# SimonMacLean/NeRF-or-nothing

Hardware: AMD Instinct MI355X
Metric: train rays/sec (128 samples/ray, 8×256 MLP) at 1/2/4/8 MI355X; PSNR vs ref (higher is better)
Workload: dtype f32; 1 GPU; BASELINE configs[1]: 1024-ray global batch x 128+128 samples, 8x256 MLP fwd/bwd + Adam; global_batch=1024, rays_per_gpu=1024, micro_batch=1024, parallelism=dp1, precision=f32

## Files before the change

nerf-or-nothing_amd/csrc/kernels/mlp16.h:

```cpp
#pragma once
#include "mlp_common.h"

namespace nof {

constexpr int kMlp16Threads = 512;
constexpr int kIpe16Floats = 6 * 64 * 4;

__device__ __forceinline__ f32x4 mfma16(float a, float b, f32x4 c) {
  return __builtin_amdgcn_mfma_f32_16x16x4f32(a, b, c, 0, 0, 0);
}

__device__ __forceinline__ void slice16_dma_step(const float* __restrict__ src, float* dst, int tid, int i) {
  const int wave = tid >> 6;
  const __amdgpu_buffer_rsrc_t rsrc =
      __builtin_amdgcn_make_buffer_rsrc(const_cast<float*>(src), (short)0, 0x7fffffff, 0x00020000);
  __builtin_amdgcn_raw_ptr_buffer_load_lds(rsrc, (lptr_t)(dst + (kMlp16Threads * i + 64 * wave) * 4), 16, tid * 16,
                                           i * kMlp16Threads * 16, 0, 0);
}
__device__ __forceinline__ void slice16_dma(const float* __restrict__ src, float* dst, int tid) {
#pragma unroll
  for (int i = 0; i < 4; ++i) slice16_dma_step(src, dst, tid, i);
}

template <int P> constexpr int ring16_slots() { return P == 0 ? 4 : 3; }
template <int P> constexpr int ring16_floats() { return ring16_slots<P>() * kSliceFloats; }
__device__ __forceinline__ void ring16_prologue(const float* __restrict__ img, float* lds, int tid) {
  slice16_dma(img, lds, tid);
  slice16_dma(img + kSliceFloats, lds + kSliceFloats, tid);
}

__device__ __forceinline__ constexpr int feat16(int t, int g, int r) { return 16 * t + 4 * g + r; }

constexpr int kStoreNT = 2;
struct BlkStore16 {
  static constexpr bool kHalf = false;
  uint32_t voff[4];
  __device__ __forceinline__ BlkStore16(int lane, int half) {
    const int g = lane >> 4, s = 16 * half + (lane & 15);
#pragma unroll
    for (int r = 0; r < 4; ++r)
      voff[r] = 512u * g + ((((s >> 2) ^ (4 * (g & 1) + r)) << 4) | ((s & 3) << 2));
  }
  __device__ __forceinline__ void store(__amdgpu_buffer_rsrc_t blk, int t, int r, float v) const {
    __builtin_amdgcn_raw_buffer_store_b32(__float_as_uint(v), blk, (int)voff[r], 2048 * t + 128 * r, kStoreNT);
  }
};
__device__ __forceinline__ __amdgpu_buffer_rsrc_t blk_rsrc(float* blk) {
  return __builtin_amdgcn_make_buffer_rsrc(blk, (short)0, 0x7fffffff, 0x00020000);
}

template <bool kNT>
struct BlkStore16H {
  static constexpr bool kHalf = true;
  uint32_t voff;
  uint32_t voff2;
  uint32_t sel;
  __device__ __forceinline__ BlkStore16H(int lane, int half) {
    const int g = lane >> 4, j = lane & 15;
    voff = 256u * g + ((((2 * half + (j >> 3)) ^ g) << 4) | ((j & 7) << 1));
    voff2 = 256u * g + 64u * (j & 1) + ((((2 * half + (j >> 3)) ^ g) << 4) | ((j & 6) << 1));
    sel = (j & 1) ? 0x03020706u : 0x05040100u;
  }
  __device__ __forceinline__ void store_pairs(__amdgpu_buffer_rsrc_t blk, int t, uint32_t p01, uint32_t p23) const {
    const uint32_t q01 = (uint32_t)__builtin_amdgcn_mov_dpp((int)p01, 0xB1, 0xF, 0xF, false);
    const uint32_t q23 = (uint32_t)__builtin_amdgcn_mov_dpp((int)p23, 0xB1, 0xF, 0xF, false);
    __builtin_amdgcn_raw_buffer_store_b32(__builtin_amdgcn_perm(q01, p01, sel), blk, (int)voff2, 1024 * t,
                                          kNT ? kStoreNT : 0);
    __builtin_amdgcn_raw_buffer_store_b32(__builtin_amdgcn_perm(q23, p23, sel), blk, (int)voff2 + 128, 1024 * t,
                                          kNT ? kStoreNT : 0);
  }
  __device__ __forceinline__ void store(__amdgpu_buffer_rsrc_t blk, int t, int r, float v) const {
    store_h(blk, t, r, (_Float16)v);
  }
  __device__ __forceinline__ void store_h(__amdgpu_buffer_rsrc_t blk, int t, int r, _Float16 h) const {
    __builtin_amdgcn_raw_buffer_store_b16(__builtin_bit_cast(unsigned short, h), blk, (int)voff + 64 * r, 1024 * t,
                                          kNT ? kStoreNT : 0);
  }
};
template <int P, bool kBwd> struct Store16 { typedef BlkStore16 T; typedef float E; };
template <bool kBwd> struct Store16<2, kBwd> { typedef BlkStore16H<true> T; typedef _Float16 E; };
template <class E>
__device__ __forceinline__ __amdgpu_buffer_rsrc_t blk_rsrc_t(E* blk) {
  return __builtin_amdgcn_make_buffer_rsrc(blk, (short)0, 0x7fffffff, 0x00020000);
}

__device__ __forceinline__ uint2* mask16_ptr(uint32_t* masks, int blk, int slot, int half, int lane) {
  return reinterpret_cast<uint2*>(mask_ptr(masks, blk, slot) + half * 128) + lane;
}
__device__ __forceinline__ bool mask16_bit(const uint2& m, int t, int r) {
  return ((t >> 3 ? m.y : m.x) >> (31 - ((t & 7) * 4 + r))) & 1u;
}
__device__ __forceinline__ float mask16_apply(const uint2& m, int t, int r, float v) {
  const uint32_t w = t >> 3 ? m.y : m.x;
  uint32_t all;
  asm("v_bfe_i32 %0, %1, %2, 1" : "=v"(all) : "v"(w), "n"(31 - ((t & 7) * 4 + r)));
  return __uint_as_float(__float_as_uint(v) & all);
}

__device__ __forceinline__ float relu_bit(float z, uint32_t& mw) {
  const int h = max(__float_as_int(z), 0);
  asm volatile("v_cmp_lt_i32 vcc, 0, %1\n\tv_addc_co_u32 %0, vcc, %0, %0, vcc" : "+v"(mw) : "v"(h) : "vcc");
  return __int_as_float(h);
}

__device__ __forceinline__ void split4h(const float (&x)[4], uint32_t& hi01, uint32_t& hi23, uint32_t& lo01,
                                        uint32_t& lo23) {
  typedef _Float16 h2 __attribute__((ext_vector_type(2)));
  typedef float f2 __attribute__((ext_vector_type(2)));
  hi01 = __builtin_bit_cast(uint32_t, __builtin_convertvector((f2{x[0], x[1]}), h2));
  hi23 = __builtin_bit_cast(uint32_t, __builtin_convertvector((f2{x[2], x[3]}), h2));
  float r[4];
  asm("v_fma_mix_f32 %0, %1, 1.0, -%2 op_sel_hi:[0,0,1]" : "=v"(r[0]) : "v"(x[0]), "v"(hi01));
  asm("v_fma_mix_f32 %0, %1, 1.0, -%2 op_sel:[0,0,1] op_sel_hi:[0,0,1]" : "=v"(r[1]) : "v"(x[1]), "v"(hi01));
  asm("v_fma_mix_f32 %0, %1, 1.0, -%2 op_sel_hi:[0,0,1]" : "=v"(r[2]) : "v"(x[2]), "v"(hi23));
  asm("v_fma_mix_f32 %0, %1, 1.0, -%2 op_sel:[0,0,1] op_sel_hi:[0,0,1]" : "=v"(r[3]) : "v"(x[3]), "v"(hi23));
  lo01 = __builtin_bit_cast(uint32_t, __builtin_convertvector((f2{r[0], r[1]}), h2));
  lo23 = __builtin_bit_cast(uint32_t, __builtin_convertvector((f2{r[2], r[3]}), h2));
}

template <bool kSplit, bool kStore, class ST>
__device__ __forceinline__ void put_tile(float (&bin)[16][4], int t, const float (&v)[4], const ST& bst,
                                         __amdgpu_buffer_rsrc_t blk) {
  if constexpr (kSplit) {
    uint32_t hi01, hi23, lo01, lo23;
    split4h(v, hi01, hi23, lo01, lo23);
    const int row = t & ~1, c = 2 * (t & 1);
    bin[row][c] = __uint_as_float(hi01);
    bin[row][c + 1] = __uint_as_float(hi23);
    bin[row + 1][c] = __uint_as_float(lo01);
    bin[row + 1][c + 1] = __uint_as_float(lo23);
    if constexpr (kStore) {
      if constexpr (ST::kHalf) {
        bst.store_pairs(blk, t, hi01, hi23);
      } else {
#pragma unroll
        for (int r = 0; r < 4; ++r) bst.store(blk, t, r, v[r]);
      }
    }
  } else {
#pragma unroll
    for (int r = 0; r < 4; ++r) {
      bin[t][r] = v[r];
      if constexpr (kStore) bst.store(blk, t, r, v[r]);
    }
  }
}

struct NoEpi16 {
  static constexpr int kVmPerPart = 0;
  __device__ __forceinline__ void operator()(int) {}
};

template <int NT_B, int NT_I, int OT, int kSlots, class Epi>
__device__ __forceinline__ void mlp_layer16(const float (&bin)[16][4], const float* ipe, f32x4 (&acc)[16],
                                            float* lds, int& cur, const float*& wsrc, bool last_in_schedule, int tid,
                                            int lane, Epi& epi, const float* cinit) {
  static_assert(OT % 2 == 0 && OT <= 16, "row tiles come in pairs");
  constexpr int NG = OT;
  constexpr int kEpiGroup1 = 4;
  constexpr int kEpiGroup2 = (NG / 2 + 4 < NG) ? NG / 2 + 4 : NG - 1;
  const int g = lane >> 4;
  const int row = lane & 15;
  const int swz = (row >> 1) & 7;
#pragma unroll
  for (int t = 0; t < NT_B + NT_I; ++t) {
    const bool dma = !(last_in_schedule && t + 2 >= NT_B + NT_I);
    const int nxt2 = kSlots == 4 ? ((cur + 2) & 3) : (cur == 0 ? 2 : cur - 1);
    const float* W = lds + cur * kSliceFloats + row * 32;
    auto aread = [&](int q, int which) {
      const int tt = q / (OT / 2), p = q % (OT / 2);
      return *reinterpret_cast<const f32x4*>(W + (2 * p + which) * 16 * 32 + (((4 * tt + g) ^ swz) << 2));
    };
    f32x4 a0 = aread(0, 0), a1 = aread(0, 1);
    auto cread = [&](int p, int which) { return *reinterpret_cast<const f32x4*>(cinit + 16 * (2 * p + which)); };
    f32x4 c0 = {}, c1 = {};
    if (t == 0 && cinit) { c0 = cread(0, 0); c1 = cread(0, 1); }
#pragma unroll
    for (int q = 0; q < NG; ++q) {
      const int tt = q / (OT / 2), p = q % (OT / 2);
      f32x4 b4;
      if (t < NT_B) {
        const int tb = (t < NT_B) ? 2 * t + tt : 0;
        b4[0] = bin[tb][0]; b4[1] = bin[tb][1]; b4[2] = bin[tb][2]; b4[3] = bin[tb][3];
      } else {
        const int ti = (t >= NT_B) ? 2 * (t - NT_B) + tt : 0;
        if constexpr (kSlots == 4) {
          b4[0] = ipe[4 * ti]; b4[1] = ipe[4 * ti + 1]; b4[2] = ipe[4 * ti + 2]; b4[3] = ipe[4 * ti + 3];
        } else b4 = *reinterpret_cast<const f32x4*>(ipe + (ti * 64 + lane) * 4);
      }
      asm volatile("" ::"v"(a0), "v"(a1), "v"(c0), "v"(c1));
      f32x4 n0 = a0, n1 = a1, m0 = c0, m1 = c1;
      if (q + 1 < NG) {
        n0 = aread(q + 1, 0);
        n1 = aread(q + 1, 1);
      }
      if (t == 0 && cinit && q + 1 < OT / 2) { m0 = cread(q + 1, 0); m1 = cread(q + 1, 1); }
      if (dma && q < 4) slice16_dma_step(wsrc + 2 * kSliceFloats, lds + nxt2 * kSliceFloats, tid, q);
      __builtin_amdgcn_sched_barrier(0);
      const bool first = t == 0 && tt == 0;
#pragma unroll
      for (int r = 0; r < 4; ++r) {
        acc[2 * p] = mfma16(a0[r], b4[r], (first && r == 0) ? c0 : acc[2 * p]);
        acc[2 * p + 1] = mfma16(a1[r], b4[r], (first && r == 0) ? c1 : acc[2 * p + 1]);
      }
      if (t + 1 < NT_B && q == kEpiGroup1) epi(2 * t + 2);
      if (t + 1 < NT_B && q == kEpiGroup2) epi(2 * t + 3);
      __builtin_amdgcn_sched_barrier(0);
      a0 = n0;
      a1 = n1;
      c0 = m0;
      c1 = m1;
    }
    if constexpr (kSlots == 4) {
      if (cur & 1) slice_barrier(t + 1 < NT_B ? 2 * Epi::kVmPerPart : 0);
      cur = (cur + 1) & 3;
    } else {
      slice_barrier((dma ? 4 : 0) + (t + 1 < NT_B ? 2 * Epi::kVmPerPart : 0));
      cur = cur == 2 ? 0 : cur + 1;
    }
    wsrc += kSliceFloats;
  }
}
template <int NT_B, int NT_I, int OT, class Epi>
__device__ __forceinline__ void mlp_layer16h(const float (&bin)[16][4], const float* ipe_lds, f32x4 (&acc)[16],
                                             float* lds, int& cur, const float*& wsrc, bool last_in_schedule, int tid,
                                             int lane, Epi& epi, const float* cinit) {
  typedef SplitMode<2> SM;
  static_assert(OT % 2 == 0 && OT <= 16, "row tiles come in pairs");
  constexpr int kPieces = 2;
  constexpr int kPP0 = 0;
  constexpr int kDmaSteps = 4;
  constexpr int kSlots = ring16_slots<2>();
  constexpr int NG = OT / 2;
  constexpr int kE1 = NG > 4 ? 4 : NG - 1;
  constexpr int kE2 = NG > 6 ? 6 : NG - 1;
#pragma unroll
  for (int t = 0; t < NT_B + NT_I; ++t) {
    const bool dma = !(last_in_schedule && t + 2 >= NT_B + NT_I);
    const int nxt2 = kSlots == 4 ? ((cur + 2) & 3) : (cur == 0 ? 2 : cur - 1);
    const f16x8* W = reinterpret_cast<const f16x8*>(lds + cur * kSliceFloats) + lane;
    Frag<2> b;
    float v[8];
    if (t < NT_B) {
      const int tb = t < NT_B ? 2 * t : 0;
      const f32x4 hi = {bin[tb][0], bin[tb][1], bin[tb][2], bin[tb][3]};
      const f32x4 lo = {bin[tb + 1][0], bin[tb + 1][1], bin[tb + 1][2], bin[tb + 1][3]};
      b.p[0] = __builtin_bit_cast(f16x8, hi);
      b.p[1] = __builtin_bit_cast(f16x8, lo);
    } else {
      const int ti = t >= NT_B ? 2 * (t - NT_B) : 0;
      if constexpr (kSlots == 4) {
#pragma unroll
        for (int i = 0; i < 8; ++i) v[i] = ipe_lds[4 * ti + i];
      } else {
        const f32x4 u0 = *reinterpret_cast<const f32x4*>(ipe_lds + (ti * 64 + lane) * 4);
        const f32x4 u1 = *reinterpret_cast<const f32x4*>(ipe_lds + ((ti + 1) * 64 + lane) * 4);
#pragma unroll
        for (int i = 0; i < 4; ++i) { v[i] = u0[i]; v[4 + i] = u1[i]; }
      }
      split8<2>(v, b);
    }
    Frag<2> a0, a1;
#pragma unroll
    for (int p = 0; p < kPieces; ++p) { a0.p[p] = W[(16 * p) * 64]; a1.p[p] = W[(16 * p + 1) * 64]; }
    auto cread = [&](int rt) { return *reinterpret_cast<const f32x4*>(cinit + 16 * rt); };
    f32x4 c0 = {}, c1 = {};
    if (t == 0 && cinit) { c0 = cread(0); c1 = cread(1); }
#pragma unroll
    for (int q = 0; q < NG; ++q) {
      if constexpr (kPieces == 2) asm volatile("" ::"v"(a0.p[0]), "v"(a0.p[1]), "v"(a1.p[0]), "v"(a1.p[1]), "v"(c0), "v"(c1));
      else asm volatile("" ::"v"(a0.p[0]), "v"(a1.p[0]), "v"(c0), "v"(c1));
      Frag<2> n0 = a0, n1 = a1;
      f32x4 m0 = c0, m1 = c1;
      if (t == 0 && cinit && q + 1 < NG) { m0 = cread(2 * q + 2); m1 = cread(2 * q + 3); }
      if (q + 1 < NG) {
#pragma unroll
        for (int p = 0; p < kPieces; ++p) {
          n0.p[p] = W[(16 * p + 2 * q + 2) * 64];
          n1.p[p] = W[(16 * p + 2 * q + 3) * 64];
        }
      }
      if (dma && q < kDmaSteps) slice16_dma_step(wsrc + 2 * kSliceFloats, lds + nxt2 * kSliceFloats, tid, q);
      __builtin_amdgcn_sched_barrier(0);
      const bool first = t == 0;
#pragma unroll
      for (int pp = kPP0; pp < SM::NPROD; ++pp) {
        acc[2 * q] = SM::mfma16(a0.p[SM::pa(pp)], b.p[SM::pb(pp)], (first && pp == kPP0) ? c0 : acc[2 * q]);
        acc[2 * q + 1] = SM::mfma16(a1.p[SM::pa(pp)], b.p[SM::pb(pp)], (first && pp == kPP0) ? c1 : acc[2 * q + 1]);
      }
      if (t + 1 < NT_B && q == kE1) epi(2 * t + 2);
      if (t + 1 < NT_B && q == kE2) epi(2 * t + 3);
      __builtin_amdgcn_sched_barrier(0);
      a0 = n0;
      a1 = n1;
      c0 = m0;
      c1 = m1;
    }
    if constexpr (kSlots == 4) {
      if (cur & 1) slice_barrier(t + 1 < NT_B ? 2 * Epi::kVmPerPart : 0);
      cur = (cur + 1) & 3;
    } else {
      slice_barrier((dma ? kDmaSteps : 0) + (t + 1 < NT_B ? 2 * Epi::kVmPerPart : 0));
      cur = cur == 2 ? 0 : cur + 1;
    }
    wsrc += kSliceFloats;
  }
}

template <int P, int NT_B, int NT_I, int OT, class Epi>
__device__ __forceinline__ void layer16(const float (&bin)[16][4], const float* ipe_lds, f32x4 (&acc)[16], float* lds,
                                        int& cur, const float*& wsrc, bool last_in_schedule, int tid, int lane,
                                        Epi& epi, const float* cinit = nullptr) {
  if constexpr (P == 2 || P == 3)
    mlp_layer16h<NT_B, NT_I, OT>(bin, ipe_lds, acc, lds, cur, wsrc, last_in_schedule, tid, lane, epi, cinit);
  else
    mlp_layer16<NT_B, NT_I, OT, ring16_slots<P>()>(bin, ipe_lds, acc, lds, cur, wsrc, last_in_schedule, tid, lane,
                                                   epi, cinit);
}
template <int P, int NT_B, int NT_I, int OT>
__device__ __forceinline__ void layer16(const float (&bin)[16][4], const float* ipe_lds, f32x4 (&acc)[16], float* lds,
                                        int& cur, const float*& wsrc, bool last_in_schedule, int tid, int lane,
                                        const float* cinit = nullptr) {
  NoEpi16 none;
  layer16<P, NT_B, NT_I, OT>(bin, ipe_lds, acc, lds, cur, wsrc, last_in_schedule, tid, lane, none, cinit);
}

}
```

nerf-or-nothing_amd/csrc/kernels/mlp_bwd16.hip:

```cpp
#include "common.h"
#include "launch.h"
#include "mlp16.h"

namespace nof {


template <bool kDensity, class ST, bool kSplit = false>
struct BwdEpi16 {
  static constexpr int kVmPerPart = 4;
  const f32x4 (&acc)[16];
  float (&bin)[16][4];
  const ST& bst;
  const int g;
  const float* w8;
  float dzs;
  __amdgpu_buffer_rsrc_t dst_blk;
  uint2 mk;
  f32x4 wnext;

  __device__ __forceinline__ BwdEpi16(const f32x4 (&acc_)[16], float (&bin_)[16][4], const ST& bst_, int lane)
      : acc(acc_), bin(bin_), bst(bst_), g(lane >> 4) {}
  template <class E>
  __device__ __forceinline__ void begin(const uint2* mask, E* dst_blk_, const float* w8_ = nullptr, float dzs_ = 0.0f) {
    mk = *mask;
    dst_blk = blk_rsrc_t(dst_blk_);
    if constexpr (kDensity) {
      w8 = w8_ + 4 * g;
      dzs = dzs_;
      wnext = *reinterpret_cast<const f32x4*>(w8);
    }
  }
  __device__ __forceinline__ void operator()(int t) {
    f32x4 w4;
    if constexpr (kDensity) {
      w4 = wnext;
      if (t + 1 < 16) wnext = *reinterpret_cast<const f32x4*>(w8 + 16 * (t + 1));
    }
    float v[4];
#pragma unroll
    for (int r = 0; r < 4; ++r) {
      v[r] = acc[t][r];
      if constexpr (kDensity) v[r] = __builtin_fmaf(w4[r], dzs, v[r]);
      v[r] = mask16_apply(mk, t, r, v[r]);
    }
    put_tile<kSplit, true>(bin, t, v, bst, dst_blk);
  }
  __device__ __forceinline__ void tile01() {
    (*this)(0);
    (*this)(1);
  }
};

template <int P>
__global__ __launch_bounds__(kMlp16Threads, 1) void k_mlp_bwd16(BwdArgs a0) {
  typedef typename Store16<P, true>::T ST;
  typedef typename Store16<P, true>::E AE;
  __shared__ __attribute__((aligned(16))) float lds[ring16_floats<P>() + 256];
  float* w8_lds = lds + ring16_floats<P>();
  const int tid = threadIdx.x, lane = tid & 63, g = lane >> 4, j = lane & 15;
  const int wave = __builtin_amdgcn_readfirstlane(tid >> 6);
  const int half = wave & 1;
  const ST bst(lane, half);
  const int wg0 = (a0.M / kBlk + 3) / 4;
  const bool second = a0.M1 > 0 && (int)blockIdx.x >= wg0;
  struct {
    int M;
    const float *dsigma, *drgb, *zhead;
    const uint32_t *amax, *masks;
    const float* wimg_b;
    float dbias, rgb_scale;
    float *delta, *delta9x;
  } a;
  a.M = second ? a0.M1 : a0.M;
  a.dsigma = second ? a0.dsigma1 : a0.dsigma;
  a.drgb = second ? a0.drgb1 : a0.drgb;
  a.zhead = second ? a0.zhead1 : a0.zhead;
  a.amax = second ? a0.amax1 : a0.amax;
  a.masks = second ? a0.masks1 : a0.masks;
  a.delta = second ? a0.delta1 : a0.delta;
  a.delta9x = second ? a0.delta9x1 : a0.delta9x;
  a.wimg_b = a0.wimg_b; a.dbias = a0.dbias; a.rgb_scale = a0.rgb_scale;
  const int wg = second ? (int)blockIdx.x - wg0 : (int)blockIdx.x;
  const int nblk = a.M / kBlk;
  const int blk_raw = wg * 4 + (wave >> 1);
  const int blk = blk_raw < nblk ? blk_raw : nblk - 1;
  const int m = blk * kBlk + 16 * half + j;
  NOF_DCHECK(a.M % kBlk == 0 && blk >= 0 && blk < nblk, kChkMlpBlock);
  const float* tail = a.wimg_b + (size_t)kBwdSlices * kSliceFloats;
  const size_t layer_stride = (size_t)nblk * kWidth * kBlk;
  uint32_t* masks = const_cast<uint32_t*>(a.masks);

  const f32x4 zh = reinterpret_cast<const f32x4*>(a.zhead)[m];
  const float dsig = a.dsigma[m];
  const float drgb3[3] = {a.drgb[(size_t)m * 3], a.drgb[(size_t)m * 3 + 1], a.drgb[(size_t)m * 3 + 2]};
  float sc = 1.0f;
  if constexpr (P >= 2) sc = delta_scale(a.amax, false);
  const uint2 mk9 = *mask16_ptr(masks, blk, 8, half, lane);
  f32x4 w10r[8][3];
#pragma unroll
  for (int t = 0; t < 8; ++t)
#pragma unroll
    for (int c = 0; c < 3; ++c)
      w10r[t][c] = *reinterpret_cast<const f32x4*>(tail + kBwdTailW10 + 128 * c + 16 * t + 4 * g);
  const f32x4 w8r = reinterpret_cast<const f32x4*>(tail + kBwdTailW8)[lane];
  __builtin_amdgcn_sched_barrier(0);
  ring16_prologue(a.wimg_b, lds, tid);
  __builtin_amdgcn_sched_barrier(0);

  float dzs = dsig * sigmoid_f(zh[0] + a.dbias);
  float dzc[3];
#pragma unroll
  for (int c = 0; c < 3; ++c) {
    const float s = sigmoid_f(zh[1 + c]);
    dzc[c] = drgb3[c] * (s * (1.0f - s)) * a.rgb_scale;
  }
  if constexpr (P >= 2) {
    dzs *= sc;
#pragma unroll
    for (int c = 0; c < 3; ++c) dzc[c] *= sc;
  }
  if (wave == 0) reinterpret_cast<f32x4*>(w8_lds)[lane] = w8r;
  const __amdgpu_buffer_rsrc_t d9 = blk_rsrc_t(reinterpret_cast<AE*>(a.delta9x) + (size_t)blk * kD9F * kBlk);
#pragma unroll
  for (int r = 0; r < 4; ++r) bst.store(d9, 8, r, g == 0 ? (r == 0 ? dzs : dzc[r - 1]) : 0.0f);
  float bin[16][4];
#pragma unroll
  for (int t = 0; t < 8; ++t) {
    float v[4];
#pragma unroll
    for (int r = 0; r < 4; ++r)
      v[r] = mask16_apply(mk9, t, r, __builtin_fmaf(w10r[t][2][r], dzc[2],
                                                   __builtin_fmaf(w10r[t][1][r], dzc[1], w10r[t][0][r] * dzc[0])));
    put_tile<P >= 2, true>(bin, t, v, bst, d9);
  }
  constexpr int kD9Stores = 4 + 8 * (P == 2 ? 2 : 4);
  static_assert(kD9Stores == (P == 2 ? 20 : 36), "the literals in the waits below");
  if constexpr (P == 2) asm volatile("s_waitcnt vmcnt(20)\n\ts_waitcnt lgkmcnt(0)\n\ts_barrier" ::: "memory");
  else asm volatile("s_waitcnt vmcnt(36)\n\ts_waitcnt lgkmcnt(0)\n\ts_barrier" ::: "memory");

  int cur = 0;
  const float* wsrc = a.wimg_b;
  f32x4 accA[16], accB[16];
  AE* delta_blk = reinterpret_cast<AE*>(a.delta) + (size_t)blk * kWidth * kBlk;
  BwdEpi16<true, ST, P >= 2> e7(accA, bin, bst, lane);
  e7.begin(mask16_ptr(masks, blk, 7, half, lane), delta_blk + 7 * layer_stride, w8_lds, dzs);
  layer16<P, 4, 0, 16>(bin, nullptr, accA, lds, cur, wsrc, false, tid, lane);
  e7.tile01();
  BwdEpi16<false, ST, P >= 2> ea(accA, bin, bst, lane), eb(accB, bin, bst, lane);
  eb.begin(mask16_ptr(masks, blk, 6, half, lane), delta_blk + 6 * layer_stride);
  layer16<P, 8, 0, 16>(bin, nullptr, accB, lds, cur, wsrc, false, tid, lane, e7);
  eb.tile01();
  static_assert(kDepth == 8, "bwd pairing assumes 8 trunk layers");
  for (int l = kDepth - 2; l >= 2; l -= 2) {
    ea.begin(mask16_ptr(masks, blk, l - 1, half, lane), delta_blk + (l - 1) * layer_stride);
    layer16<P, 8, 0, 16>(bin, nullptr, accA, lds, cur, wsrc, false, tid, lane, eb);
    ea.tile01();
    eb.begin(mask16_ptr(masks, blk, l - 2, half, lane), delta_blk + (l - 2) * layer_stride);
    layer16<P, 8, 0, 16>(bin, nullptr, accB, lds, cur, wsrc, l == 2, tid, lane, ea);
    eb.tile01();
  }
#pragma unroll
  for (int t = 2; t < 16; ++t) eb(t);
}

hipError_t launch_mlp_bwd16(const BwdArgs& a, hipStream_t st) {
  const dim3 grid((a.M / kBlk + 3) / 4 + (a.M1 > 0 ? (a.M1 / kBlk + 3) / 4 : 0));
  if (a.split == 2) hipLaunchKernelGGL(k_mlp_bwd16<2>, grid, dim3(kMlp16Threads), 0, st, a);
  else if (a.split == 3) hipLaunchKernelGGL(k_mlp_bwd16<3>, grid, dim3(kMlp16Threads), 0, st, a);
  else hipLaunchKernelGGL(k_mlp_bwd16<0>, grid, dim3(kMlp16Threads), 0, st, a);
  return hipGetLastError();
}

NOF_CHECK_UNIT(check_unit_mlp_bwd16)

}
```

nerf-or-nothing_amd/csrc/kernels/mlp_fwd16.hip:

```cpp
#include "common.h"
#include "geometry.h"
#include "launch.h"
#include "mlp16.h"

namespace nof {


template <bool store, bool kDensity, int NT, class ST, bool kSplit = false>
struct FwdEpi16 {
  static constexpr int kVmPerPart = store ? 4 : 0;
  const f32x4 (&acc)[16];
  float (&bin)[16][4];
  const ST& bst;
  const int g;
  const float* w8;
  __amdgpu_buffer_rsrc_t act_blk;
  uint2* mask_dst;
  uint32_t mw[2];
  f32x4 wnext;
  float zs;

  __device__ __forceinline__ FwdEpi16(const f32x4 (&acc_)[16], float (&bin_)[16][4], const ST& bst_, int lane)
      : acc(acc_), bin(bin_), bst(bst_), g(lane >> 4) {}
  template <class E>
  __device__ __forceinline__ void begin(E* act_blk_, uint2* mask_dst_, const float* w8_ = nullptr) {
    act_blk = blk_rsrc_t(act_blk_);
    mask_dst = mask_dst_;
    mw[0] = mw[1] = 0u;
    if constexpr (kDensity) {
      w8 = w8_ + 4 * g;
      wnext = *reinterpret_cast<const f32x4*>(w8);
      zs = 0.0f;
    }
  }
  __device__ __forceinline__ void operator()(int t) {
    const bool more = t + 1 < NT;
    f32x4 w4;
    if constexpr (kDensity) {
      w4 = wnext;
      if (more) wnext = *reinterpret_cast<const f32x4*>(w8 + 16 * (t + 1));
    }
    float hv[4];
#pragma unroll
    for (int r = 0; r < 4; ++r) {
      hv[r] = relu_bit(acc[t][r], mw[t >> 3]);
      if constexpr (kDensity) zs = __builtin_fmaf(w4[r], hv[r], zs);
    }
    put_tile<kSplit, store>(bin, t, hv, bst, act_blk);
    if constexpr (store && kVmPerPart > 0)
      if (!more) *mask_dst = make_uint2(mw[0], mw[1]);
  }
  __device__ __forceinline__ void tile01() {
    (*this)(0);
    (*this)(1);
  }
};

template <int P, bool store>
__global__ __launch_bounds__(kMlp16Threads, 1) void k_mlp_fwd16(FwdArgs a) {
  typedef typename Store16<P, false>::T ST;
  typedef typename Store16<P, false>::E AE;
  constexpr int kRing = ring16_slots<P>() * kSliceFloats;
  constexpr bool kIpeReg = ring16_slots<P>() == 4;
  constexpr int kIpeLds = kIpeReg ? 0 : 8 * kIpe16Floats;
  constexpr int kBiasLds = 8 * 256 + 256;
  __shared__ __attribute__((aligned(16))) float lds[kRing + kIpeLds + 8 * 128 + kBiasLds];
  const int tid = threadIdx.x, lane = tid & 63, g = lane >> 4, j = lane & 15;
  const int wave = __builtin_amdgcn_readfirstlane(tid >> 6);
  const int half = wave & 1;
  const int nblk = a.M / kBlk;
  const int blk_raw = blockIdx.x * 4 + (wave >> 1);
  const int blk = blk_raw < nblk ? blk_raw : nblk - 1;
  const int m0 = blk * kBlk;
  const int ray = m0 / a.S;
  const int s0 = m0 - ray * a.S + 16 * half;
  const int m = m0 + 16 * half + j;
  const float* tail = a.wimg + (size_t)kFwdSlices * kSliceFloats;
  NOF_DCHECK(a.M % kBlk == 0 && a.S % kBlk == 0 && blk >= 0 && blk < nblk, kChkMlpBlock);

  const bool vtab = a.view_pe != nullptr;
  float t01[2] = {0.0f, 0.0f};
  float d3[3] = {0.0f, 0.0f, 0.0f}, o3[3] = {0.0f, 0.0f, 0.0f}, radius = 0.0f;
  if (!a.encoded) {
    const float* tr = a.t + (size_t)ray * (a.S + 1) + s0 + j;
    t01[0] = tr[0]; t01[1] = tr[1];
    d3[0] = a.dirs[3 * ray]; d3[1] = a.dirs[3 * ray + 1]; d3[2] = a.dirs[3 * ray + 2];
    o3[0] = a.origins[3 * ray]; o3[1] = a.origins[3 * ray + 1]; o3[2] = a.origins[3 * ray + 2];
    radius = a.radii[ray];
  }
  f32x4 vpe[2] = {};
  float vb[2] = {0.0f, 0.0f};
  if (vtab) {
#pragma unroll
    for (int u = 0; u < 2; ++u)
      vpe[u] = *reinterpret_cast<const f32x4*>(a.view_pe + (size_t)ray * 32 + (feat16(6 + u, g, 0) - kPosIn));
#pragma unroll
    for (int rep = 0; rep < 2; ++rep) vb[rep] = a.view_bias[(size_t)ray * 128 + lane + 64 * rep];
  }
  static_assert(kBiasLds / 4 > kMlp16Threads && kBiasLds / 4 <= kMlp16Threads + 64, "bias table: wave 0 takes the rest");
  const f32x4 tab0 = *reinterpret_cast<const f32x4*>(tail + kFwdTailBias + 4 * tid);
  f32x4 tab1 = {};
  if (wave == 0) tab1 = *reinterpret_cast<const f32x4*>(tail + kFwdTailW8 + 4 * tid);
  __builtin_amdgcn_sched_barrier(0);
  ring16_prologue(a.wimg, lds, tid);
  __builtin_amdgcn_sched_barrier(0);

  float ipe[6][4];
  if (!a.encoded) {
    float mean[3], cov[3];
    frustum_gaussian(t01[0], t01[1], o3, d3, radius, mean, cov, a.cylinder != 0);
#pragma unroll
    for (int t = 0; t < 6; ++t)
#pragma unroll
      for (int r = 0; r < 4; ++r)
        ipe[t][r] = ipe_feature(feat16(t, g, r), mean, cov);
  } else {
#pragma unroll
    for (int t = 0; t < 6; ++t)
#pragma unroll
      for (int r = 0; r < 4; ++r) ipe[t][r] = a.enc_pos[(size_t)m * kPosIn + feat16(t, g, r)];
#pragma unroll
    for (int t = 0; t < 6; ++t)
#pragma unroll
      for (int r = 0; r < 4; ++r) asm volatile("" : "+v"(ipe[t][r]));
  }
  float pe[kDirIn];
  if (!vtab) {
    const int kl = lane < kDirIn ? lane : 0;
    const float pe_l = a.encoded ? a.enc_dir[(size_t)ray * kDirIn + kl] : dir_feature(kl, d3);
#pragma unroll
    for (int k = 0; k < kDirIn; ++k) pe[k] = __int_as_float(__builtin_amdgcn_readlane(__float_as_int(pe_l), k));
  }
  const float* ipe_b = &ipe[0][0];
  if constexpr (!kIpeReg) {
    float* ipe_lds = lds + kRing + wave * kIpe16Floats;
#pragma unroll
    for (int t = 0; t < 6; ++t) {
      f32x4 v;
      v[0] = ipe[t][0]; v[1] = ipe[t][1]; v[2] = ipe[t][2]; v[3] = ipe[t][3];
      *reinterpret_cast<f32x4*>(ipe_lds + (t * 64 + lane) * 4) = v;
    }
    ipe_b = ipe_lds;
  }
  float* dirb = lds + kRing + kIpeLds + wave * 128;
  float* bias_lds = lds + kRing + kIpeLds + 8 * 128;
  *reinterpret_cast<f32x4*>(bias_lds + 4 * tid) = tab0;
  if (wave == 0) *reinterpret_cast<f32x4*>(bias_lds + 4 * (kMlp16Threads + tid)) = tab1;
  if (vtab) {
#pragma unroll
    for (int rep = 0; rep < 2; ++rep) dirb[lane + 64 * rep] = vb[rep];
  } else {
#pragma unroll
    for (int rep = 0; rep < 2; ++rep) {
      const int o = lane + 64 * rep;
      float s = tail[kFwdTailBias + 9 * 256 + o];
      const float* w9 = tail + kFwdTailW9d + o * 32;
#pragma unroll
      for (int k = 0; k < kDirIn; ++k) s = __builtin_fmaf(w9[k], pe[k], s);
      dirb[o] = s;
    }
  }

  const ST bst(lane, half);
  if constexpr (store) {
    float vrow[2][4];
    if (vtab) {
#pragma unroll
      for (int u = 0; u < 2; ++u)
#pragma unroll
        for (int r = 0; r < 4; ++r) vrow[u][r] = vpe[u][r];
    } else {
#pragma unroll
      for (int u = 0; u < 2; ++u)
#pragma unroll
        for (int r = 0; r < 4; ++r) {
          const int k = feat16(6 + u, g, r) - kPosIn;
          float v = 0.0f;
#pragma unroll
          for (int kk = 0; kk < kDirIn; ++kk) v = (kk == k) ? pe[kk] : v;
          vrow[u][r] = v;
        }
    }
    __builtin_amdgcn_sched_barrier(0);
    const __amdgpu_buffer_rsrc_t act_in_rs = blk_rsrc_t(reinterpret_cast<AE*>(a.act_in) + (size_t)blk * kInF * kBlk);
#pragma unroll
    for (int t = 0; t < 6; ++t)
#pragma unroll
      for (int r = 0; r < 4; ++r) bst.store(act_in_rs, t, r, ipe[t][r]);
#pragma unroll
    for (int u = 0; u < 2; ++u)
#pragma unroll
      for (int r = 0; r < 4; ++r) bst.store(act_in_rs, 6 + u, r, vrow[u][r]);
    constexpr int kActInStores = 8 * 4;
    static_assert(kActInStores == 32 && kActInStores < 64, "the literal in the wait below");
    asm volatile("s_waitcnt vmcnt(32)\n\ts_waitcnt lgkmcnt(0)\n\ts_barrier" ::: "memory");
  } else {
    __syncthreads();
  }

  int cur = 0;
  const float* wsrc = a.wimg;
  f32x4 accA[16], accB[16];
  float bin[16][4];
  const size_t layer_stride = (size_t)nblk * kWidth * kBlk;
  const float* biases = bias_lds;
  AE* act_h_blk = reinterpret_cast<AE*>(a.act_h) + (size_t)blk * kWidth * kBlk;

  constexpr bool kPre = P >= 2;
  FwdEpi16<store, false, 16, ST, kPre> ea(accA, bin, bst, lane), eb(accB, bin, bst, lane);
  const float* bias_g = biases + 4 * g;
  ea.begin(act_h_blk, mask16_ptr(a.masks, blk, 0, half, lane));
  layer16<P, 0, 3, 16>(bin, ipe_b, accA, lds, cur, wsrc, false, tid, lane, bias_g);
  ea.tile01();
  for (int l = 1; l < kDepth - 1; l += 2) {
    eb.begin(act_h_blk + l * layer_stride, mask16_ptr(a.masks, blk, l, half, lane));
    layer16<P, 8, 0, 16>(bin, ipe_b, accB, lds, cur, wsrc, false, tid, lane, ea, bias_g + l * 256);
    eb.tile01();
    ea.begin(act_h_blk + (l + 1) * layer_stride, mask16_ptr(a.masks, blk, l + 1, half, lane));
    if (l + 1 == kSkip)
      layer16<P, 8, 3, 16>(bin, ipe_b, accA, lds, cur, wsrc, false, tid, lane, eb, bias_g + (l + 1) * 256);
    else layer16<P, 8, 0, 16>(bin, ipe_b, accA, lds, cur, wsrc, false, tid, lane, eb, bias_g + (l + 1) * 256);
    ea.tile01();
  }
  static_assert(kDepth == 8 && kSkip % 2 == 0, "trunk pairing assumes 8 layers and an even skip layer");
  FwdEpi16<store, true, 16, ST, kPre> e7(accB, bin, bst, lane);
  e7.begin(act_h_blk + 7 * layer_stride, mask16_ptr(a.masks, blk, 7, half, lane), bias_lds + 8 * 256);
  layer16<P, 8, 0, 16>(bin, ipe_b, accB, lds, cur, wsrc, false, tid, lane, ea, bias_g + 7 * 256);
  e7.tile01();

  layer16<P, 8, 0, 8>(bin, ipe_b, accA, lds, cur, wsrc, true, tid, lane, e7, dirb + 4 * g);
  float zs = e7.zs;
  zs += __shfl_xor(zs, 16, 64);
  zs += __shfl_xor(zs, 32, 64);
  zs += tail[kFwdTailBias + 8 * 256];
  FwdEpi16<store, false, 8, ST> e9(accA, bin, bst, lane);
  e9.begin(reinterpret_cast<AE*>(a.act_h9) + (size_t)blk * kWidthCond * kBlk, mask16_ptr(a.masks, blk, 8, half, lane));
#pragma unroll
  for (int t = 0; t < 8; ++t) e9(t);

  float zc[3] = {0.0f, 0.0f, 0.0f};
#pragma unroll
  for (int c = 0; c < 3; ++c) {
#pragma unroll
    for (int t = 0; t < 8; ++t) {
      const f32x4 w4 = *reinterpret_cast<const f32x4*>(tail + kFwdTailW10 + c * 128 + 16 * t + 4 * g);
#pragma unroll
      for (int r = 0; r < 4; ++r) zc[c] = __builtin_fmaf(w4[r], bin[t][r], zc[c]);
    }
    zc[c] += __shfl_xor(zc[c], 16, 64);
    zc[c] += __shfl_xor(zc[c], 32, 64);
    zc[c] += tail[kFwdTailBias + 10 * 256 + c];
  }

  if (g == 0) {
    a.sigma[m] = softplus_f(zs + a.dbias);
#pragma unroll
    for (int c = 0; c < 3; ++c) a.rgb[(size_t)m * 3 + c] = sigmoid_f(zc[c]) * a.rgb_scale - a.rgb_pad;
    f32x4 zh;
    zh[0] = zs; zh[1] = zc[0]; zh[2] = zc[1]; zh[3] = zc[2];
    if constexpr (store) reinterpret_cast<f32x4*>(a.zhead)[m] = zh;
  }
}

hipError_t launch_mlp_fwd16(const FwdArgs& a, hipStream_t st) {
  const int nblk = a.M / kBlk;
  const dim3 grid((nblk + 3) / 4), block(kMlp16Threads);
  if (a.split == 2) {
    if (a.no_store) hipLaunchKernelGGL((k_mlp_fwd16<2, false>), grid, block, 0, st, a);
    else hipLaunchKernelGGL((k_mlp_fwd16<2, true>), grid, block, 0, st, a);
  } else if (a.split == 3) {
    if (a.no_store) hipLaunchKernelGGL((k_mlp_fwd16<2, false>), grid, block, 0, st, a);
    else hipLaunchKernelGGL((k_mlp_fwd16<3, true>), grid, block, 0, st, a);
  } else {
    if (a.no_store) hipLaunchKernelGGL((k_mlp_fwd16<0, false>), grid, block, 0, st, a);
    else hipLaunchKernelGGL((k_mlp_fwd16<0, true>), grid, block, 0, st, a);
  }
  return hipGetLastError();
}

NOF_CHECK_UNIT(check_unit_mlp_fwd16)

}
```

Measured before the change: 166,400 rays/s.

## Overlap layer seam epilogues with final slice MFMAs and stage head weights in LDS

Moves the epilogue of each layer's first output tiles (and most of the last head layer's tiles) into the final weight slice's MFMA loop, where they used to run serially after the layer. The slice barrier on the final slice is skipped and its wait count adjusted for the new in-flight stores. Separately, the forward kernel now stages the W10 head weights and the head biases into LDS with the bias table, replacing global tail reads. The cost is more complex scheduling, tighter vmcnt accounting and extra LDS use.

```diff
diff --git a/nerf-or-nothing_amd/csrc/kernels/mlp16.h b/nerf-or-nothing_amd/csrc/kernels/mlp16.h
--- a/nerf-or-nothing_amd/csrc/kernels/mlp16.h
+++ b/nerf-or-nothing_amd/csrc/kernels/mlp16.h
@@ -151,14 +151,26 @@
   __device__ __forceinline__ void operator()(int) {}
 };
 
-template <int NT_B, int NT_I, int OT, int kSlots, class Epi>
+#ifndef NOF_SEAM_OWN_TILES
+#define NOF_SEAM_OWN_TILES 1
+#endif
+#ifndef NOF_SEAM_HEAD_LDS
+#define NOF_SEAM_HEAD_LDS 1
+#endif
+
+template <int NT_B, int NT_I, int OT, int kSlots, int kOwn, class Epi, class Own>
 __device__ __forceinline__ void mlp_layer16(const float (&bin)[16][4], const float* ipe, f32x4 (&acc)[16],
                                             float* lds, int& cur, const float*& wsrc, bool last_in_schedule, int tid,
-                                            int lane, Epi& epi, const float* cinit) {
+                                            int lane, Epi& epi, Own& own, const float* cinit) {
   static_assert(OT % 2 == 0 && OT <= 16, "row tiles come in pairs");
+  static_assert(kOwn == 0 || kOwn == 2 || kOwn == OT - 2, "own tiles: none, the first pair, or all but the last pair");
+  static_assert(kOwn == 0 || NT_I > 0 || NT_B == 0 || kOwn <= 2 * NT_B - 2, "the bin argument above");
+  constexpr bool kOwnIn = NOF_SEAM_OWN_TILES && kOwn > 0;
   constexpr int NG = OT;
   constexpr int kEpiGroup1 = 4;
   constexpr int kEpiGroup2 = (NG / 2 + 4 < NG) ? NG / 2 + 4 : NG - 1;
+  constexpr int kOwnGroup0 = OT / 2 + 2, kOwnGroup1 = OT / 2 + 5;
+  static_assert(kOwn != 2 || (kOwnGroup1 < NG && kOwnGroup0 > 4), "own tiles 0, 1: behind the DMA steps, inside the slice");
   const int g = lane >> 4;
   const int row = lane & 15;
   const int swz = (row >> 1) & 7;
@@ -205,6 +217,17 @@
       }
       if (t + 1 < NT_B && q == kEpiGroup1) epi(2 * t + 2);
       if (t + 1 < NT_B && q == kEpiGroup2) epi(2 * t + 3);
+      if constexpr (kOwnIn) {
+        if (t + 1 == NT_B + NT_I) {
+          if constexpr (kOwn == 2) {
+            if (q == kOwnGroup0) own(0);
+            if (q == kOwnGroup1) own(1);
+          } else {
+            const int p2 = q - (OT / 2 + 1);
+            if (p2 >= 0 && 2 * p2 + 1 < kOwn) { own(2 * p2); own(2 * p2 + 1); }
+          }
+        }
+      }
       __builtin_amdgcn_sched_barrier(0);
       a0 = n0;
       a1 = n1;
@@ -212,13 +235,20 @@
       c1 = m1;
     }
     if constexpr (kSlots == 4) {
-      if (cur & 1) slice_barrier(t + 1 < NT_B ? 2 * Epi::kVmPerPart : 0);
+      constexpr int own_vm = kOwnIn ? kOwn * Own::kVmPerPart : 0;
+      const bool final_slice = NOF_SEAM_OWN_TILES && last_in_schedule && t + 1 == NT_B + NT_I;
+      if ((cur & 1) && !final_slice)
+        slice_barrier((t + 1 < NT_B ? 2 * Epi::kVmPerPart : 0) + (t + 1 == NT_B + NT_I ? own_vm : 0));
       cur = (cur + 1) & 3;
     } else {
       slice_barrier((dma ? 4 : 0) + (t + 1 < NT_B ? 2 * Epi::kVmPerPart : 0));
       cur = cur == 2 ? 0 : cur + 1;
     }
     wsrc += kSliceFloats;
+  }
+  if constexpr (!kOwnIn) {
+#pragma unroll
+    for (int u = 0; u < kOwn; ++u) own(u);
   }
 }
 template <int NT_B, int NT_I, int OT, class Epi>
@@ -307,22 +337,25 @@
   }
 }
 
-template <int P, int NT_B, int NT_I, int OT, class Epi>
+template <int P, int NT_B, int NT_I, int OT, int kOwn, class Epi, class Own>
 __device__ __forceinline__ void layer16(const float (&bin)[16][4], const float* ipe_lds, f32x4 (&acc)[16], float* lds,
                                         int& cur, const float*& wsrc, bool last_in_schedule, int tid, int lane,
-                                        Epi& epi, const float* cinit = nullptr) {
-  if constexpr (P == 2 || P == 3)
+                                        Epi& epi, Own& own, const float* cinit = nullptr) {
+  if constexpr (P == 2 || P == 3) {
     mlp_layer16h<NT_B, NT_I, OT>(bin, ipe_lds, acc, lds, cur, wsrc, last_in_schedule, tid, lane, epi, cinit);
-  else
-    mlp_layer16<NT_B, NT_I, OT, ring16_slots<P>()>(bin, ipe_lds, acc, lds, cur, wsrc, last_in_schedule, tid, lane,
-                                                   epi, cinit);
-}
-template <int P, int NT_B, int NT_I, int OT>
-__device__ __forceinline__ void layer16(const float (&bin)[16][4], const float* ipe_lds, f32x4 (&acc)[16], float* lds,
-                                        int& cur, const float*& wsrc, bool last_in_schedule, int tid, int lane,
-                                        const float* cinit = nullptr) {
+#pragma unroll
+    for (int u = 0; u < kOwn; ++u) own(u);
+  } else {
+    mlp_layer16<NT_B, NT_I, OT, ring16_slots<P>(), kOwn>(bin, ipe_lds, acc, lds, cur, wsrc, last_in_schedule, tid,
+                                                         lane, epi, own, cinit);
+  }
+}
+template <int P, int NT_B, int NT_I, int OT, int kOwn, class Own>
+__device__ __forceinline__ void layer16_first(const float (&bin)[16][4], const float* ipe_lds, f32x4 (&acc)[16],
+                                              float* lds, int& cur, const float*& wsrc, int tid, int lane, Own& own,
+                                              const float* cinit = nullptr) {
   NoEpi16 none;
-  layer16<P, NT_B, NT_I, OT>(bin, ipe_lds, acc, lds, cur, wsrc, last_in_schedule, tid, lane, none, cinit);
-}
-
-}
+  layer16<P, NT_B, NT_I, OT, kOwn>(bin, ipe_lds, acc, lds, cur, wsrc, false, tid, lane, none, own, cinit);
+}
+
+}
diff --git a/nerf-or-nothing_amd/csrc/kernels/mlp_bwd16.hip b/nerf-or-nothing_amd/csrc/kernels/mlp_bwd16.hip
--- a/nerf-or-nothing_amd/csrc/kernels/mlp_bwd16.hip
+++ b/nerf-or-nothing_amd/csrc/kernels/mlp_bwd16.hip
@@ -44,10 +44,6 @@
       v[r] = mask16_apply(mk, t, r, v[r]);
     }
     put_tile<kSplit, true>(bin, t, v, bst, dst_blk);
-  }
-  __device__ __forceinline__ void tile01() {
-    (*this)(0);
-    (*this)(1);
   }
 };
 
@@ -144,23 +140,23 @@
   AE* delta_blk = reinterpret_cast<AE*>(a.delta) + (size_t)blk * kWidth * kBlk;
   BwdEpi16<true, ST, P >= 2> e7(accA, bin, bst, lane);
   e7.begin(mask16_ptr(masks, blk, 7, half, lane), delta_blk + 7 * layer_stride, w8_lds, dzs);
-  layer16<P, 4, 0, 16>(bin, nullptr, accA, lds, cur, wsrc, false, tid, lane);
-  e7.tile01();
+  layer16_first<P, 4, 0, 16, 2>(bin, nullptr, accA, lds, cur, wsrc, tid, lane, e7);
   BwdEpi16<false, ST, P >= 2> ea(accA, bin, bst, lane), eb(accB, bin, bst, lane);
   eb.begin(mask16_ptr(masks, blk, 6, half, lane), delta_blk + 6 * layer_stride);
-  layer16<P, 8, 0, 16>(bin, nullptr, accB, lds, cur, wsrc, false, tid, lane, e7);
-  eb.tile01();
+  layer16<P, 8, 0, 16, 2>(bin, nullptr, accB, lds, cur, wsrc, false, tid, lane, e7, eb);
   static_assert(kDepth == 8, "bwd pairing assumes 8 trunk layers");
-  for (int l = kDepth - 2; l >= 2; l -= 2) {
+  for (int l = kDepth - 2; l >= 4; l -= 2) {
     ea.begin(mask16_ptr(masks, blk, l - 1, half, lane), delta_blk + (l - 1) * layer_stride);
-    layer16<P, 8, 0, 16>(bin, nullptr, accA, lds, cur, wsrc, false, tid, lane, eb);
-    ea.tile01();
+    layer16<P, 8, 0, 16, 2>(bin, nullptr, accA, lds, cur, wsrc, false, tid, lane, eb, ea);
     eb.begin(mask16_ptr(masks, blk, l - 2, half, lane), delta_blk + (l - 2) * layer_stride);
-    layer16<P, 8, 0, 16>(bin, nullptr, accB, lds, cur, wsrc, l == 2, tid, lane, ea);
-    eb.tile01();
+    layer16<P, 8, 0, 16, 2>(bin, nullptr, accB, lds, cur, wsrc, false, tid, lane, ea, eb);
   }
-#pragma unroll
-  for (int t = 2; t < 16; ++t) eb(t);
+  ea.begin(mask16_ptr(masks, blk, 1, half, lane), delta_blk + layer_stride);
+  layer16<P, 8, 0, 16, 2>(bin, nullptr, accA, lds, cur, wsrc, false, tid, lane, eb, ea);
+  eb.begin(mask16_ptr(masks, blk, 0, half, lane), delta_blk);
+  layer16<P, 8, 0, 16, 14>(bin, nullptr, accB, lds, cur, wsrc, true, tid, lane, ea, eb);
+  eb(14);
+  eb(15);
 }
 
 hipError_t launch_mlp_bwd16(const BwdArgs& a, hipStream_t st) {
diff --git a/nerf-or-nothing_amd/csrc/kernels/mlp_fwd16.hip b/nerf-or-nothing_amd/csrc/kernels/mlp_fwd16.hip
--- a/nerf-or-nothing_amd/csrc/kernels/mlp_fwd16.hip
+++ b/nerf-or-nothing_amd/csrc/kernels/mlp_fwd16.hip
@@ -50,10 +50,6 @@
     if constexpr (store && kVmPerPart > 0)
       if (!more) *mask_dst = make_uint2(mw[0], mw[1]);
   }
-  __device__ __forceinline__ void tile01() {
-    (*this)(0);
-    (*this)(1);
-  }
 };
 
 template <int P, bool store>
@@ -63,7 +59,10 @@
   constexpr int kRing = ring16_slots<P>() * kSliceFloats;
   constexpr bool kIpeReg = ring16_slots<P>() == 4;
   constexpr int kIpeLds = kIpeReg ? 0 : 8 * kIpe16Floats;
-  constexpr int kBiasLds = 8 * 256 + 256;
+  constexpr bool kHeadLds = NOF_SEAM_HEAD_LDS;
+  constexpr int kHeadW10 = 0, kHeadB8 = 384, kHeadB10 = 388, kHeadFloats = kHeadLds ? 392 : 0;
+  constexpr int kBiasLds = 8 * 256 + 256 + kHeadFloats;
+  static_assert(kFwdTailW10 == kFwdTailW8 + 256, "w8 and W10 are one contiguous run of the image's tail");
   __shared__ __attribute__((aligned(16))) float lds[kRing + kIpeLds + 8 * 128 + kBiasLds];
   const int tid = threadIdx.x, lane = tid & 63, g = lane >> 4, j = lane & 15;
   const int wave = __builtin_amdgcn_readfirstlane(tid >> 6);
@@ -97,10 +96,17 @@
 #pragma unroll
     for (int rep = 0; rep < 2; ++rep) vb[rep] = a.view_bias[(size_t)ray * 128 + lane + 64 * rep];
   }
-  static_assert(kBiasLds / 4 > kMlp16Threads && kBiasLds / 4 <= kMlp16Threads + 64, "bias table: wave 0 takes the rest");
+  static_assert(kBiasLds / 4 > kMlp16Threads && kBiasLds / 4 <= 2 * kMlp16Threads, "bias table: two chunks per thread");
   const f32x4 tab0 = *reinterpret_cast<const f32x4*>(tail + kFwdTailBias + 4 * tid);
   f32x4 tab1 = {};
-  if (wave == 0) tab1 = *reinterpret_cast<const f32x4*>(tail + kFwdTailW8 + 4 * tid);
+  constexpr int kTab1 = kBiasLds / 4 - kMlp16Threads;
+  if constexpr (kHeadLds) {
+    static_assert(kTab1 == 162 && 8 * 256 + 256 + kHeadB8 == 4 * (kMlp16Threads + 160) && kHeadB10 == kHeadB8 + 4, "chunk map");
+    const int src = tid < 160 ? kFwdTailW8 + 4 * tid : (tid == 160 ? kFwdTailBias + 8 * 256 : kFwdTailBias + 10 * 256);
+    tab1 = *reinterpret_cast<const f32x4*>(tail + src);
+  } else {
+    if (wave == 0) tab1 = *reinterpret_cast<const f32x4*>(tail + kFwdTailW8 + 4 * tid);
+  }
   __builtin_amdgcn_sched_barrier(0);
   ring16_prologue(a.wimg, lds, tid);
   __builtin_amdgcn_sched_barrier(0);
@@ -145,7 +151,8 @@
   float* dirb = lds + kRing + kIpeLds + wave * 128;
   float* bias_lds = lds + kRing + kIpeLds + 8 * 128;
   *reinterpret_cast<f32x4*>(bias_lds + 4 * tid) = tab0;
-  if (wave == 0) *reinterpret_cast<f32x4*>(bias_lds + 4 * (kMlp16Threads + tid)) = tab1;
+  if (kHeadLds ? tid < kTab1 : wave == 0) *reinterpret_cast<f32x4*>(bias_lds + 4 * (kMlp16Threads + tid)) = tab1;
+  const float* head_lds = bias_lds + 8 * 256 + 256;
   if (vtab) {
 #pragma unroll
     for (int rep = 0; rep < 2; ++rep) dirb[lane + 64 * rep] = vb[rep];
@@ -210,46 +217,44 @@
   FwdEpi16<store, false, 16, ST, kPre> ea(accA, bin, bst, lane), eb(accB, bin, bst, lane);
   const float* bias_g = biases + 4 * g;
   ea.begin(act_h_blk, mask16_ptr(a.masks, blk, 0, half, lane));
-  layer16<P, 0, 3, 16>(bin, ipe_b, accA, lds, cur, wsrc, false, tid, lane, bias_g);
-  ea.tile01();
+  layer16_first<P, 0, 3, 16, 2>(bin, ipe_b, accA, lds, cur, wsrc, tid, lane, ea, bias_g);
   for (int l = 1; l < kDepth - 1; l += 2) {
     eb.begin(act_h_blk + l * layer_stride, mask16_ptr(a.masks, blk, l, half, lane));
-    layer16<P, 8, 0, 16>(bin, ipe_b, accB, lds, cur, wsrc, false, tid, lane, ea, bias_g + l * 256);
-    eb.tile01();
+    layer16<P, 8, 0, 16, 2>(bin, ipe_b, accB, lds, cur, wsrc, false, tid, lane, ea, eb, bias_g + l * 256);
     ea.begin(act_h_blk + (l + 1) * layer_stride, mask16_ptr(a.masks, blk, l + 1, half, lane));
     if (l + 1 == kSkip)
-      layer16<P, 8, 3, 16>(bin, ipe_b, accA, lds, cur, wsrc, false, tid, lane, eb, bias_g + (l + 1) * 256);
-    else layer16<P, 8, 0, 16>(bin, ipe_b, accA, lds, cur, wsrc, false, tid, lane, eb, bias_g + (l + 1) * 256);
-    ea.tile01();
+      layer16<P, 8, 3, 16, 2>(bin, ipe_b, accA, lds, cur, wsrc, false, tid, lane, eb, ea, bias_g + (l + 1) * 256);
+    else layer16<P, 8, 0, 16, 2>(bin, ipe_b, accA, lds, cur, wsrc, false, tid, lane, eb, ea, bias_g + (l + 1) * 256);
   }
   static_assert(kDepth == 8 && kSkip % 2 == 0, "trunk pairing assumes 8 layers and an even skip layer");
   FwdEpi16<store, true, 16, ST, kPre> e7(accB, bin, bst, lane);
   e7.begin(act_h_blk + 7 * layer_stride, mask16_ptr(a.masks, blk, 7, half, lane), bias_lds + 8 * 256);
-  layer16<P, 8, 0, 16>(bin, ipe_b, accB, lds, cur, wsrc, false, tid, lane, ea, bias_g + 7 * 256);
-  e7.tile01();
-
-  layer16<P, 8, 0, 8>(bin, ipe_b, accA, lds, cur, wsrc, true, tid, lane, e7, dirb + 4 * g);
+  layer16<P, 8, 0, 16, 2>(bin, ipe_b, accB, lds, cur, wsrc, false, tid, lane, ea, e7, bias_g + 7 * 256);
+
+  FwdEpi16<store, false, 8, ST> e9(accA, bin, bst, lane);
+  e9.begin(reinterpret_cast<AE*>(a.act_h9) + (size_t)blk * kWidthCond * kBlk, mask16_ptr(a.masks, blk, 8, half, lane));
+  layer16<P, 8, 0, 8, 6>(bin, ipe_b, accA, lds, cur, wsrc, true, tid, lane, e7, e9, dirb + 4 * g);
   float zs = e7.zs;
   zs += __shfl_xor(zs, 16, 64);
   zs += __shfl_xor(zs, 32, 64);
-  zs += tail[kFwdTailBias + 8 * 256];
-  FwdEpi16<store, false, 8, ST> e9(accA, bin, bst, lane);
-  e9.begin(reinterpret_cast<AE*>(a.act_h9) + (size_t)blk * kWidthCond * kBlk, mask16_ptr(a.masks, blk, 8, half, lane));
-#pragma unroll
-  for (int t = 0; t < 8; ++t) e9(t);
-
+  zs += kHeadLds ? head_lds[kHeadB8] : tail[kFwdTailBias + 8 * 256];
+  e9(6);
+  e9(7);
+
+  const float* w10 = kHeadLds ? head_lds + kHeadW10 : tail + kFwdTailW10;
+  const float* b10 = kHeadLds ? head_lds + kHeadB10 : tail + kFwdTailBias + 10 * 256;
   float zc[3] = {0.0f, 0.0f, 0.0f};
 #pragma unroll
   for (int c = 0; c < 3; ++c) {
 #pragma unroll
     for (int t = 0; t < 8; ++t) {
-      const f32x4 w4 = *reinterpret_cast<const f32x4*>(tail + kFwdTailW10 + c * 128 + 16 * t + 4 * g);
+      const f32x4 w4 = *reinterpret_cast<const f32x4*>(w10 + c * 128 + 16 * t + 4 * g);
 #pragma unroll
       for (int r = 0; r < 4; ++r) zc[c] = __builtin_fmaf(w4[r], bin[t][r], zc[c]);
     }
     zc[c] += __shfl_xor(zc[c], 16, 64);
     zc[c] += __shfl_xor(zc[c], 32, 64);
-    zc[c] += tail[kFwdTailBias + 10 * 256 + c];
+    zc[c] += b10[c];
   }
 
   if (g == 0) {
```

Result: no change. 167,800 rays/s, median of 6 (+0.8%).
